# saza-ku/kube-scheduler-simulator

Measured on AMD Instinct MI355X. Metric: pods scheduled/sec @5k nodes, default plugins; node-evals/sec; % HBM peak, higher is better.
Workload: dtype int64

## Files before the change

### kube-scheduler-simulator_amd/csrc/ksched.hip

```cpp
#include <hip/hip_runtime.h>

#include <algorithm>
#include <atomic>
#include <chrono>
#include <array>
#include <cstdio>
#include <cstring>
#include <mutex>
#include <set>
#include <string>
#include <tuple>
#include <type_traits>
#include <vector>

#include "ksched_kernels.h"

#include "ksched_dev.h"
#include "ksched_json_host.h"

using namespace ksk;

#include "ksched_parts.h"

struct ksg_ctx {
// ... 671 lines not shown
    if ((rc = decide_n32(ctx, first, count, &n32))) return rc;
  }
  b.stat = n32 ? ctx->d_stat : nullptr;
  ctx->last_spec = false;
  ctx->last_mw = false;
  (void)hipGetLastError();
  treset(ctx);
  HIPC(ctx, hipEventRecord(ctx->ev0, ctx->stream));
  int trc;
  if ((trc = tmark(ctx))) return trc;
  for (int off = 0; off < count;) {
    int nb = std::min(ctx->slot_block, count - off);
    int64_t lo = 0, hi = 0;
    size_t bytes = 0;
    const size_t budget = kLdsBudget;
    for (;;) {
      lo = ctx->h_pods[first + off].blob;
      hi = lo;
      for (int k = 0; k < nb; k++) {
        const ksg_pod& q = ctx->h_pods[first + off + k];
        lo = std::min<int64_t>(lo, q.blob);
        hi = std::max<int64_t>(hi, (int64_t)q.blob + q.blob_len);
      }
      const size_t words = (cm_words + (size_t)nb * (sizeof(ksg_pod) / 4) + (size_t)(hi - lo) + 3) & ~(size_t)3;
      bytes = 4 * words + (size_t)nb * slot_bytes;
      if (bytes <= budget || nb == 1) break;
      nb = std::max(1, nb / 2);
    }
    if (bytes > budget) return fail(ctx, KSG_E_UNSUPPORTED, "batch does not fit the LDS budget");
    b.b0 = first + off;
    b.out0 = off;
    b.nb = nb;
    b.prog_lo = (int32_t)lo;
    b.prog_len = (int32_t)(hi - lo);
    const double units = (double)b.nb * N;
    hipLaunchKernelGGL(ksg_batch_phase1, dim3((N + 255) / 256, b.nb), dim3(256), 0, ctx->stream, b);
    if ((trc = tlaunched(ctx, KSG_K_BATCH_PHASE1, units))) return trc;
    hipLaunchKernelGGL(ksg_batch_topk<1024>, dim3(b.nb), dim3(1024), 0, ctx->stream, b);
    if ((trc = tlaunched(ctx, KSG_K_BATCH_TOPK, units))) return trc;
    hipLaunchKernelGGL(reinterpret_cast<void (*)(BatchArgs)>(
                           const_cast<void*>(slot_kernels()[slot_kernel_index(n32, slot_rm, ctx->slot_block)])),
                       dim3(1), dim3(ctx->slot_block), bytes, ctx->stream, b);
    if ((trc = tlaunched(ctx, KSG_K_BATCH_PHASE2S, 0.5 * b.nb * (b.nb + 1)))) return trc;
    if (cap) {
      CapArgs ca = *cap;
      ca.b0 = b.b0;
      ca.nb = b.nb;
      ca.out0 = b.out0;
      ca.rec = ctx->d_rec;
      HIPC(ctx, hipMemsetAsync(ca.stats, 0, sizeof(int32_t) * 4 * b.nb, ctx->stream));
      hipLaunchKernelGGL(ksg_capture_eval, dim3((N + 255) / 256, b.nb), dim3(256), 0, ctx->stream, ca);
      if ((trc = tlaunched(ctx, KSG_K_CAPTURE_EVAL, units))) return trc;
      hipLaunchKernelGGL(ksg_capture_norm, dim3((N + 255) / 256, b.nb), dim3(256), 0, ctx->stream, ca);
      if ((trc = tlaunched(ctx, KSG_K_CAPTURE_NORM, units))) return trc;
    }
    off += nb;
  }
  HIPC(ctx, hipGetLastError());
  HIPC(ctx, hipEventRecord(ctx->ev1, ctx->stream));
  return KSG_OK;
}

int state_copy(ksg_ctx* ctx, bool save);

int run_spec_persistent(ksg_ctx* ctx, const BatchArgs& b0, int32_t first, int32_t count, size_t cm_words, bool mw,
                        unsigned* tk, int32_t* carry_n) {
  const int N = ctx->c.N;
  constexpr int B = 64;
  std::vector<int32_t>& tab = ctx->h_btab;
  tab.clear();
  for (int off = 0, prev_nb = 0; off < count;) {
    int nb = std::min(B, count - off);
    int64_t lo = 0, hi = 0;
    size_t bytes = 0;
    for (;;) {
      lo = ctx->h_pods[first + off].blob;
      hi = lo;
      for (int k = 0; k < nb; k++) {
        const ksg_pod& q = ctx->h_pods[first + off + k];
        lo = std::min<int64_t>(lo, q.blob);
        hi = std::max<int64_t>(hi, (int64_t)q.blob + q.blob_len);
      }
      bytes = 4 * ((cm_words + (size_t)nb * (sizeof(ksg_pod) / 4) + (size_t)(hi - lo) + 3) & ~(size_t)3) +
              (size_t)kSvSlots * kSvRow * 8 + (size_t)kSvSlots * 64 * 4 + (size_t)64 * (nb + prev_nb) * 4;
      if (bytes <= kSpecLds || nb == 1) break;
      nb = std::max(1, nb / 2);
    }
    if (bytes > kSpecLds) return fail(ctx, KSG_E_UNSUPPORTED, "batch does not fit the LDS budget");
    for (int32_t v : {first + off, off, nb, (int32_t)lo, (int32_t)(hi - lo), prev_nb}) tab.push_back(v);
    prev_nb = nb;
    off += nb;
  }
  const int nbatch = (int)(tab.size() / 6);
  int rc;
  if (tab.size() > ctx->btab_cap) {
    if (ctx->d_btab) {
      auto it = std::find(ctx->allocs.begin(), ctx->allocs.end(), (void*)ctx->d_btab);
      if (it != ctx->allocs.end()) ctx->allocs.erase(it);
      HIPC(ctx, hipStreamSynchronize(ctx->stream));
      (void)hipFree(ctx->d_btab);
      ctx->d_btab = nullptr;
    }
    if ((rc = dalloc(ctx, &ctx->d_btab, tab.size()))) return rc;
    ctx->btab_cap = tab.size();
  }
  if (!ctx->h_p2done) {
    HIPC(ctx, hipHostMalloc((void**)&ctx->h_p2done, 64, hipHostMallocMapped | hipHostMallocCoherent));
    void* dp = nullptr;
    HIPC(ctx, hipHostGetDevicePointer(&dp, ctx->h_p2done, 0));
    ctx->d_p2done = static_cast<unsigned*>(dp);
  }
  hipStream_t s1 = ctx->stream2, s2 = ctx->stream;
  if ((rc = state_copy(ctx, true))) return rc;
  ctx->last_persist = true;
  HIPC(ctx, hipMemcpyAsync(ctx->d_btab, tab.data(), sizeof(int32_t) * tab.size(), hipMemcpyHostToDevice, s2));
  if (ctx->inject_timeout & 16) {
    ctx->inject_timeout &= ~16;
    HIPC(ctx, hipMemsetAsync(tk + 2, 0x01, 1, s2));
  }
  volatile unsigned* done = ctx->h_p2done;
  *done = 0;
  std::atomic_thread_fence(std::memory_order_seq_cst);
  SpecRun r{};
  r.btab = ctx->d_btab;
  r.nbatch = nbatch;
  for (int q = 0; q < 2; q++) {
    r.rec[q] = ctx->d_prec[q];
    r.img[q] = ctx->d_pimg[q];
    r.rect[q] = ctx->d_prect[q];
    r.imgt[q] = ctx->d_pimgt[q];
    r.pmax[q] = ctx->d_ppmax[q];
    r.p1[q] = ctx->d_pp1[q];
    r.top[q] = ctx->d_ptop[q];
  }
  r.carry = ctx->d_carry;
  r.carry_n = carry_n;
  r.done = ctx->d_p2done;
  BatchArgs base = b0;
  base.tk_arrive = tk;
  base.tk_done = tk + 1;
  base.tk_timeout = tk + 2;
  base.walk_err = tk + 3;
  base.inject_walk_err = ctx->inject_walk_err;
  base.tk_sc = 1;
  base.stat = nullptr;
  base.xcd_grid = 1;
  const void* run_kern = mw ? (const void*)ksg_batch_phase2v_run<64 * kSvWaves, true>
                            : (const void*)ksg_batch_phase2v_run<64 * kSvWaves, false>;
  if ((rc = func_lds_attr(ctx, run_kern, kSpecLds))) return rc;
  void* kargs[] = {&base, &r};
  HIPC(ctx, hipLaunchKernel(run_kern, dim3(1), dim3(64 * kSvWaves), kargs, kSpecLds, s2));
  const auto t0 = std::chrono::steady_clock::now();
  for (int bi = 0; bi < nbatch; bi++) {
    if (bi >= 2) {
      for (unsigned spins = 0; *done < (unsigned)(bi - 1); spins++) {
        __builtin_ia32_pause();
        if ((spins & 4095) == 4095) {
          const hipError_t e = hipStreamQuery(s2);
          if (e != hipErrorNotReady && *done < (unsigned)(bi - 1)) {
            if (e != hipSuccess) return fail(ctx, KSG_E_DEVICE, std::string("spec walk: ") + hipGetErrorString(e));
            bi = nbatch;
            break;
          }
          if (std::chrono::duration<double>(std::chrono::steady_clock::now() - t0).count() > 120.0)
            return fail(ctx, KSG_E_DEVICE, "spec walk: no progress for 120 s");
        }
      }
// ... 46 lines not shown
    }
    if ((rc = dalloc(ctx, &ctx->d_carry, (size_t)2 * KSG_BATCH_MAX + 6))) return rc;
  }
  if (!ctx->stream2) {
    int least = 0, greatest = 0;
    HIPC(ctx, hipDeviceGetStreamPriorityRange(&least, &greatest));
    HIPC(ctx, hipStreamCreateWithPriority(&ctx->stream2, hipStreamNonBlocking, greatest));
    for (int q = 0; q < 2; q++) {
      HIPC(ctx, hipEventCreateWithFlags(&ctx->ev_tk[q], hipEventDisableTiming));
      HIPC(ctx, hipEventCreateWithFlags(&ctx->ev_p2[q], hipEventDisableTiming));
    }
  }
  int32_t* carry_n = ctx->d_carry + 2 * KSG_BATCH_MAX;
  unsigned* tk = reinterpret_cast<unsigned*>(carry_n + 2);
  ctx->pipe_tk = tk;
  HIPC(ctx, hipMemsetAsync(carry_n, 0, 6 * sizeof(int32_t), ctx->stream));
  const bool window = ctx->pipe_window != 0;
  const bool overlap = window && !ctx->timing && ctx->pipe_overlap;
  const int slot_rm = ctx->c.R <= 4 ? 4 : KSG_MAX_RES;
  bool n32 = false, mw = false;
  if (ctx->batch_mode >= 4 && (rc = decide_n32(ctx, first, count, &n32))) return rc;
  if (ctx->batch_mode == 6 && window && !n32 && spec_candidate(ctx) && (rc = decide_mw(ctx, first, count, &mw)))
    return rc;
  const bool specw = ctx->batch_mode == 6 && window && (n32 || mw) && spec_candidate(ctx);
  ctx->last_spec = specw;
  ctx->last_mw = specw && mw;
  const void* spec_kern = mw ? (const void*)ksg_batch_phase2v<64 * kSvWaves, true>
                             : (const void*)ksg_batch_phase2v<64 * kSvWaves, false>;
  if (specw && !ctx->d_prect[0]) {
    for (int q = 0; q < 2; q++) {
      if ((rc = dalloc(ctx, &ctx->d_prect[q], (size_t)64 * N))) return rc;
      if ((rc = dalloc(ctx, &ctx->d_pimgt[q], (size_t)64 * N))) return rc;
    }
  }
  if (specw && (rc = func_lds_attr(ctx, spec_kern, kSpecLds))) return rc;
  const int B = specw || window ? 64 : ctx->slot_block;
  const int slots = window ? 2 * B : B;
  const int sblock = slots <= 64 ? 64 : 128;
  const void* kern = slot_kernels()[slot_kernel_index(n32, slot_rm, sblock)];
  const int block = sblock;
  const size_t kLdsBudget = specw ? kSpecLds : 120 * 1024;
  const size_t slot_bytes = 8 * (size_t)(2 * slot_rm + 10);
  if ((rc = set_phase2_attrs(ctx, 120 * 1024))) return rc;
  BatchArgs b{};
  b.c = ctx->c;
  b.st = ctx->st;
  b.pods = ctx->d_pods;
  b.prog = ctx->d_prog;
  b.prof = d_prof;
  b.placements = d_pl;
  b.results = d_res;
  const size_t cm_words = (size_t)((((N + 31) / 32) + 3) & ~3);
#ifdef KSG_STAMPS
  if (!ctx->d_stamps) {
    if ((rc = dalloc(ctx, &ctx->d_stamps, 16))) return rc;
    HIPC(ctx, hipMemsetAsync(ctx->d_stamps, 0, 128, ctx->stream));
  }
  b.stamps = ctx->d_stamps;
#endif
  hipStream_t s1 = overlap ? ctx->stream2 : ctx->stream, s2 = ctx->stream;
  (void)hipGetLastError();
  treset(ctx);
  HIPC(ctx, hipEventRecord(ctx->ev0, s2));
  if (overlap) HIPC(ctx, hipStreamWaitEvent(s1, ctx->ev0, 0));
  if ((rc = tmark(ctx))) return rc;
  if (specw && overlap && ctx->spec_persist)
    return run_spec_persistent(ctx, b, first, count, cm_words, mw, tk, carry_n);
  int prev_nb = 0;
  for (int off = 0, bi = 0; off < count; bi++) {
    const int par = bi & 1;
    int nb = std::min(B, count - off);
    int64_t lo = 0, hi = 0;
    size_t bytes = 0;
    for (;;) {
      lo = ctx->h_pods[first + off].blob;
      hi = lo;
      for (int k = 0; k < nb; k++) {
        const ksg_pod& q = ctx->h_pods[first + off + k];
        lo = std::min<int64_t>(lo, q.blob);
        hi = std::max<int64_t>(hi, (int64_t)q.blob + q.blob_len);
      }
      if (specw)
        bytes = 4 * ((cm_words + (size_t)nb * (sizeof(ksg_pod) / 4) + (size_t)(hi - lo) + 3) & ~(size_t)3) +
                (size_t)kSvSlots * kSvRow * 8 + (size_t)kSvSlots * 64 * 4 + (size_t)64 * (nb + prev_nb) * 4;
      else
        bytes = 4 * ((cm_words + (size_t)nb * (sizeof(ksg_pod) / 4) + (size_t)(hi - lo) + 3) & ~(size_t)3) +
                (size_t)sblock * slot_bytes;
      if (bytes <= kLdsBudget || nb == 1) break;
      nb = std::max(1, nb / 2);
    }
    if (bytes > kLdsBudget) return fail(ctx, KSG_E_UNSUPPORTED, "batch does not fit the LDS budget");
    b.b0 = first + off;
    b.out0 = off;
    b.nb = nb;
    b.prog_lo = (int32_t)lo;
    b.prog_len = (int32_t)(hi - lo);
    b.rec = ctx->d_prec[par];
    b.img = ctx->d_pimg[par];
    b.stat = n32 && !specw ? ctx->d_pstat[par] : nullptr;
    b.rect = specw ? ctx->d_prect[par] : nullptr;
    b.imgt = specw ? ctx->d_pimgt[par] : nullptr;
    b.xcd_grid = specw ? 1 : 0;
    b.pmax = ctx->d_ppmax[par];
    b.p1 = ctx->d_pp1[par];
    b.top = ctx->d_ptop[par];
    b.k_extra = window ? prev_nb : 0;
    b.carry = window ? ctx->d_carry + (par ^ 1) * KSG_BATCH_MAX : nullptr;
    b.carry_n = window ? carry_n + (par ^ 1) : nullptr;
    b.carry_out = window ? ctx->d_carry + par * KSG_BATCH_MAX : nullptr;
    b.carry_out_n = window ? carry_n + par : nullptr;
    const double units = (double)nb * N;
    const bool tk_flag = overlap;
    b.tk_arrive = tk_flag ? tk : nullptr;
    b.tk_done = tk_flag ? tk + 1 : nullptr;
    b.tk_timeout = tk_flag ? tk + 2 : nullptr;
    b.walk_err = tk + 3;
    b.inject_walk_err = ctx->inject_walk_err;
    b.tk_seq = (unsigned)bi + 1;
    BatchArgs bt = b;
    bt.tk_sc = specw && tk_flag ? 1 : 0;
    b.tk_sc = bt.tk_sc;
    if (overlap && bi >= 2) HIPC(ctx, hipStreamWaitEvent(s1, ctx->ev_p2[par], 0));
    if (specw)
      hipLaunchKernelGGL(ksg_batch_phase1, dim3(((((N + 255) / 256) + 7) & ~7) * nb), dim3(256), 0, s1, b);
    else
      hipLaunchKernelGGL(ksg_batch_phase1, dim3((N + 255) / 256, nb), dim3(256), 0, s1, b);
    if ((rc = tlaunched(ctx, KSG_K_BATCH_PHASE1, units))) return rc;
    hipLaunchKernelGGL(ksg_batch_topk<1024>, dim3(nb), dim3(1024), 0, s1, bt);
    if ((rc = tlaunched(ctx, KSG_K_BATCH_TOPK, units))) return rc;
    if (specw) {
      hipLaunchKernelGGL(reinterpret_cast<void (*)(BatchArgs)>(const_cast<void*>(spec_kern)), dim3(1),
                         dim3(64 * kSvWaves), kSpecLds, s2, b);
      if ((rc = tlaunched(ctx, KSG_K_BATCH_PHASE2V, 0.5 * nb * (nb + 1)))) return rc;
    } else {
      hipLaunchKernelGGL(reinterpret_cast<void (*)(BatchArgs)>(const_cast<void*>(kern)), dim3(1), dim3(block), bytes, s2, b);
      if ((rc = tlaunched(ctx, KSG_K_BATCH_PHASE2S, 0.5 * nb * (nb + 1)))) return rc;
    }
    if (overlap) HIPC(ctx, hipEventRecord(ctx->ev_p2[par], s2));
    prev_nb = nb;
    off += nb;
  }
  HIPC(ctx, hipGetLastError());
  HIPC(ctx, hipEventRecord(ctx->ev1, s2));
  return KSG_OK;
}

bool sweep_eligible(ksg_ctx* ctx, const ksg_profile* profiles, int R, int first, int count) {
  if (ctx->c.T > 255) return false;
  if (range_has_ports(ctx, first, count)) return false;
  for (int r = 0; r < R; r++) {
    const ksg_profile& prof = profiles[r];
    if (needs_topo(ctx, prof, first, count)) return false;
    int64_t wsum = 0;
    for (int pl : {KSG_PL_NODE_RESOURCES_FIT, KSG_PL_BALANCED_ALLOCATION, KSG_PL_IMAGE_LOCALITY})
      if ((prof.score_mask >> pl) & 1u) {
        if (prof.weight[pl] < 0) return false;
        wsum += prof.weight[pl];
      }
    if (wsum * 100 >= (1ll << 31)) return false;
  }
  for (int i = first; i < first + count; i++)
    if (ctx->h_na_pref_sum[i] > 0xffff || ctx->h_na_pref_sum[i] < 0) return false;
  return true;
}

template <int BLOCK, bool MULTI>
hipError_t launch_one(const void* f, const SweepArgs& s, int grid, hipStream_t st) {
// ... 2819 lines not shown
```

### kube-scheduler-simulator_amd/csrc/ksched_phase2v.h

```cpp

constexpr int kSvWaves = 12;
constexpr int kSvSlots = 2 * 64;
constexpr int kSvRow = SlotLayout<4>::STRIDE;
constexpr int kSvTotalBits = 27;
constexpr int kSvOwner = 2048;

__device__ __forceinline__ bool sv_changed(const uint32_t* cm, int n) { return ((cm[n >> 5] >> (n & 31)) & 1u) != 0; }

__device__ __forceinline__ uint32_t sv_word(int32_t total, bool live, bool p1f, bool ft, bool fa) {
  return ((uint32_t)total & ((1u << kSvTotalBits) - 1)) | (live ? 1u << 27 : 0u) | (p1f ? 1u << 28 : 0u) |
         (ft ? 1u << 29 : 0u) | (fa ? 1u << 30 : 0u) | (1u << 31);
}

struct SvItem {
  int32_t node, slot, v;
  int32_t src;
  int32_t t;
};

template <int BLOCK, bool MW = false>
__device__ __forceinline__ void spec_walk_batch(const BatchArgs& a) {
  using SL = SlotLayout<4>;
  constexpr int NW = BLOCK / 64;
  constexpr int SW = SL::W;
  static_assert(BLOCK == 64 * kSvWaves && SW == 16, "spec walk layout");
  extern __shared__ __attribute__((aligned(16))) int32_t s_dyn[];
  __shared__ ksg_profile s_prof;
  __shared__ __attribute__((aligned(16))) TcU s_u[64];
  __shared__ ksg_result s_res[64];
  __shared__ int32_t s_clist[kSvSlots];
  __shared__ int32_t s_lastv[kSvSlots];
  __shared__ int32_t s_vt[kSvSlots];
  __shared__ int32_t s_dec[64];
  __shared__ uint64_t s_bu[64];
  __shared__ uint64_t s_best[64];
  __shared__ uint32_t s_cnt[64];
  __shared__ uint8_t s_snap[64 * 64];
  __shared__ uint8_t s_mstep[64];
  __shared__ uint8_t s_dptr[64];
  __shared__ uint32_t s_owner[kSvOwner];
  __shared__ SvItem s_item[64 + 1];
  __shared__ int32_t s_ctl[8];
  __shared__ P1Stats s_p1[64];

  const int tid = threadIdx.x, lane = tid & 63, wv = tid >> 6;
  const DevCluster& c = a.c;
  const int N = c.N, R = c.R;
  const int nb = a.nb;
  const int cm_words = (((N + 31) / 32) + 3) & ~3;
  constexpr int POD_WORDS = sizeof(ksg_pod) / 4;
  const int KT = nb + a.k_extra;
  uint32_t* s_cmask = reinterpret_cast<uint32_t*>(s_dyn);
  ksg_pod* s_pods = reinterpret_cast<ksg_pod*>(s_dyn + cm_words);
  int32_t* s_prog = s_dyn + cm_words + nb * POD_WORDS;
  int64_t* s_vrow = reinterpret_cast<int64_t*>(s_dyn + ((cm_words + nb * POD_WORDS + a.prog_len + 3) & ~3));
  uint32_t* s_col = reinterpret_cast<uint32_t*>(s_vrow + (size_t)kSvSlots * kSvRow);
  int32_t* s_top = reinterpret_cast<int32_t*>(s_col + (size_t)kSvSlots * 64);

#ifdef KSG_STAMPS
  unsigned long long st_acc[16] = {}, st_last = __builtin_amdgcn_s_memtime();
#endif
  if (a.tk_done) {
    if (tid == 0) {
      using G1 = __attribute__((address_space(1))) unsigned;
      unsigned spins = 0;
      while (__hip_atomic_load((G1*)a.tk_done, __ATOMIC_RELAXED, __HIP_MEMORY_SCOPE_AGENT) < a.tk_seq) {
        __builtin_amdgcn_s_sleep(2);
        if (++spins > (1u << 24)) {
          __hip_atomic_store((G1*)a.tk_timeout, 1u, __ATOMIC_RELAXED, __HIP_MEMORY_SCOPE_AGENT);
          break;
        }
      }
    }
    __syncthreads();
    __builtin_amdgcn_fence(__ATOMIC_ACQUIRE, "agent");
  }
  KSG_STAMP(8);
  for (int i = tid; i < cm_words; i += BLOCK) s_cmask[i] = 0;
  for (int i = tid; i < kSvOwner; i += BLOCK) s_owner[i] = 0xffffffffu;
  {
    constexpr int PI = (64 * POD_WORDS + BLOCK - 1) / BLOCK;
    int32_t pw[PI];
#pragma unroll
    for (int it = 0; it < PI; it++) {
      const int i = tid + it * BLOCK;
      pw[it] = i < nb * POD_WORDS ? reinterpret_cast<const int32_t*>(a.pods + a.b0)[i] : 0;
    }
#pragma unroll
    for (int it = 0; it < PI; it++) {
      const int i = tid + it * BLOCK;
      if (i < nb * POD_WORDS) reinterpret_cast<int32_t*>(s_pods)[i] = pw[it];
    }
  }
  for (int i0 = 0; i0 < a.prog_len; i0 += 4 * BLOCK) {
    int32_t g[4];
#pragma unroll
    for (int it = 0; it < 4; it++) {
      const int i = i0 + tid + it * BLOCK;
      g[it] = i < a.prog_len ? a.prog[a.prog_lo + i] : 0;
    }
#pragma unroll
    for (int it = 0; it < 4; it++) {
      const int i = i0 + tid + it * BLOCK;
      if (i < a.prog_len) s_prog[i] = g[it];
    }
  }
  for (int i = tid; i < (int)(sizeof(ksg_profile) / 4); i += BLOCK)
    reinterpret_cast<int32_t*>(&s_prof)[i] = reinterpret_cast<const int32_t*>(a.prof)[i];
  bool fit_filter_on = false;
  for (int kf = 0; kf < a.prof->n_filter; kf++) fit_filter_on |= a.prof->filter_order[kf] == KSG_PL_NODE_RESOURCES_FIT;
  {
    const int KP = (KT + 1) >> 1;
    constexpr int TI = (64 * kSvSlots / 2 + BLOCK - 1) / BLOCK;
    ulonglong2 kp[TI];
#pragma unroll
    for (int it = 0; it < TI; it++) {
      const int x = tid + it * BLOCK, q = x / KP, i = 2 * (x - q * KP);
      const uint64_t* tp = a.top + (size_t)q * KSG_BATCH_MAX + i;
      if (x >= nb * KP) kp[it] = ulonglong2{0, 0};
      else if (a.tk_sc) kp[it] = ulonglong2{ld_sc(tp), ld_sc(tp + 1)};
      else kp[it] = *reinterpret_cast<const ulonglong2*>(tp);
    }
#pragma unroll
    for (int it = 0; it < TI; it++) {
      const int x = tid + it * BLOCK, q = x / KP, i = 2 * (x - q * KP);
      if (x < nb * KP) {
        s_top[q * KT + i] = key_node(kp[it].x);
        if (i + 1 < KT) s_top[q * KT + i + 1] = key_node(kp[it].y);
      }
    }
  }
  if (tid < nb * (int)(sizeof(P1Stats) / 4)) {
    const int32_t* src = reinterpret_cast<const int32_t*>(a.p1) + tid;
    reinterpret_cast<int32_t*>(s_p1)[tid] = a.tk_sc ? ld_sc(src) : *src;
  }
  KSG_STAMP(9);
  const int nc0 = a.carry ? *a.carry_n : 0;
  if (tid < 64) {
    const int d = a.carry && tid < nc0 ? a.carry[tid] : 0;
    if (tid < nc0) {
      s_clist[tid] = d;
      s_lastv[tid] = tid;
      s_vt[tid] = -1;
      s_item[tid] = SvItem{d, tid, tid, -1, -1};
    }
  }
  __syncthreads();
  const ksg_profile& prof = s_prof;
  const TcProf cm = tc_prof(cm_prof(prof));
  if (tid < nc0) atomicOr(&s_cmask[s_clist[tid] >> 5], 1u << (s_clist[tid] & 31));
  if (wv == 0 && lane < nb) {
    const bool ipa_filter = ipa_in_filter(prof);
    const bool ipa_score = ((prof.score_mask >> KSG_PL_INTER_POD_AFFINITY) & 1u) != 0;
    const ksg_pod& p = s_pods[lane];
    const P1Stats s1 = s_p1[lane];
    const uint32_t smask = prof.score_mask & ~p.score_skip;
    TcU u;
#pragma unroll
    for (int r = 0; r < 4; r++) u.req[r] = r < R ? p.req[r] : 0;
    u.nzc = p.nz_cpu;
    u.nzm = p.nz_mem;
    u.nfeas = s1.nfeas;
    u.K = s1.K;
    u.ht = s1.ht;
    u.ha = s1.ha;
    const bool wt = (smask & bit(KSG_PL_TAINT_TOLERATION)) && prof.weight[KSG_PL_TAINT_TOLERATION];
    const bool wa = (smask & bit(KSG_PL_NODE_AFFINITY)) && prof.weight[KSG_PL_NODE_AFFINITY];
    u.flags = (s1.err ? 1u : 0u) | (wt ? 2u : 0u) | (wa ? 4u : 0u) | (p.commit >= 0 ? 8u : 0u);
    const bool ipa_none = p.ipa < 0;
    const bool ps_skip = ipa_none && ipa_score && !((p.score_skip >> KSG_PL_INTER_POD_AFFINITY) & 1u);
    u.st_pf = ipa_none && ipa_filter ? KSG_ST_IPA_PREFILTER_SKIP : 0u;
    u.st_sc = KSG_ST_SCORED | (ps_skip ? KSG_ST_IPA_PRESCORE_SKIP : 0u);
    u.skip = p.score_skip;
    u.skip_sc = p.score_skip | (ps_skip ? bit(KSG_PL_INTER_POD_AFFINITY) : 0u);
    u.pad[0] = u.pad[1] = u.pad[2] = 0;
    s_u[lane] = u;
  }
  if (tid == 0) {
    s_ctl[0] = 0;
    s_ctl[1] = nc0;
    s_ctl[2] = nc0;
    s_ctl[3] = nc0;
    s_ctl[4] = 0;
    s_ctl[6] = 0;
  }
  __syncthreads();
  for (int q = wv; q < nb; q += NW) {
    const int K = s_u[q].K;
    int ptr = K;
    for (int b = 0; b < K && ptr == K; b += 64) {
      const int i = b + lane;
      const int n = i < K ? s_top[q * KT + i] : -1;
      const uint64_t m = __ballot(i < K && !sv_changed(s_cmask, n));
      if (m) ptr = b + __builtin_ctzll(m);
    }
    if (lane == 0) s_dptr[q] = (uint8_t)ptr;
  }
  __syncthreads();

  auto delta_word = [&](const TcU& u, int w) -> int64_t {
    const int rl = (w >> 1) & 3;
    const int64_t req_l = rl == 0 ? u.req[0] : rl == 1 ? u.req[1] : rl == 2 ? u.req[2] : u.req[3];
    return w < 8 ? ((w & 1) ? req_l : 0) : w == SL::NZC ? u.nzc : w == SL::NZM ? u.nzm : w == SL::PODS ? 1 : 0;
  };
  const int qq = lane < nb ? lane : 0;
  const TcPod hp = tc_pod(s_pods[qq], prof, s_p1[qq], fit_filter_on, R);
  struct Pending {
    SvItem it;
    uint64_t x;
    int32_t st;
    int64_t wd;
  };
  auto issue = [&](const SvItem& it) -> Pending {
    Pending p{it, 0, 0, 0};
    if (it.node < 0) return p;
    if (a.inject_walk_err && lane == 0 && it.node >= 0) {
      using G1 = __attribute__((address_space(1))) unsigned;
      __hip_atomic_store((G1*)a.walk_err, 3u, __ATOMIC_RELAXED, __HIP_MEMORY_SCOPE_AGENT);
    }
    if (it.node >= N) {
      p.it.node = -1;
      if (lane == 0) {
        using G1 = __attribute__((address_space(1))) unsigned;
        __hip_atomic_store((G1*)a.walk_err, 3u, __ATOMIC_RELAXED, __HIP_MEMORY_SCOPE_AGENT);
      }
      return p;
    }
    p.x = a.rect[(size_t)it.node * 64 + lane];
    p.st = a.imgt[(size_t)it.node * 64 + lane];
    const int wl = lane < SW ? lane : 0;
    p.wd = it.src >= 0 ? s_vrow[(size_t)it.src * kSvRow + wl]
                       : slot_word_value<4, true>(slot_word_fetch<4, true>(c, a.st, wl, R, it.node), wl, R);
    return p;
  };
  auto finish = [&](const Pending& p) {
    const SvItem& it = p.it;
    if (it.node < 0) return;
    if (lane < SW) s_vrow[(size_t)it.v * kSvRow + lane] = p.wd + (it.t >= 0 ? delta_word(s_u[it.t], lane) : 0);
    int64_t w[SW];
    {
      const int4* src = reinterpret_cast<const int4*>(s_vrow + (size_t)it.v * kSvRow);
#pragma unroll
      for (int k = 0; k < SW / 2; k++) reinterpret_cast<int4*>(w)[k] = src[k];
    }
    const TcRow row = tc_row<MW>(cm, w);
    const bool p1f = (p.x >> 63) != 0;
    const bool ft = p1f && (int32_t)((p.x >> 48) & 0xff) == hp.mt;
    const bool fa = p1f && (int32_t)((p.x >> 32) & 0xffff) == hp.ma;
    const int32_t rt = (int32_t)((p.x >> 48) & 0xff), ra = (int32_t)((p.x >> 32) & 0xffff);
    const int32_t nt = hp.mt != 0 ? 100 - qdiv32(100 * rt, hp.mt, hp.inv_mt) : 100;
    const int32_t na = hp.ma != 0 ? qdiv32(100 * ra, hp.ma, hp.inv_ma) : ra;
    const int32_t stat = p.st + hp.wt * nt + hp.wa * na;
    int32_t fb = 0;
    const bool live = tc_eval<MW>(cm, hp, row, fb) && p1f;
    if (lane > it.t) s_col[it.slot * 64 + lane] = sv_word(stat + fb, live, p1f, ft, fa);
    else if (it.src < 0) s_col[it.slot * 64 + lane] = 0u;
  };

  int ptr = 0, cnode = -1, nnode = -1;
  if (wv == 0 && lane < nb) {
    ptr = s_dptr[lane];
    const int K = s_u[lane].K;
    cnode = ptr < K ? s_top[lane * KT + ptr] : -1;
    nnode = ptr + 1 < K ? s_top[lane * KT + ptr + 1] : -1;
  }
  int start = 0, nv_c = nc0, ns_c = nc0, nspecial = nc0;
  int guard = 0;
  KSG_STAMP(0);
  while (start < nb && guard++ <= nb) {
#ifdef KSG_STAMPS
    if (tid == 0) st_acc[15] += 1;
#endif
    if (wv == 0) {
      __builtin_amdgcn_s_setprio(3);
      if (lane >= start && lane < nb) {
        s_best[lane] = 0;
        s_cnt[lane] = 0;
      }
      const int Kq = lane < nb ? s_u[lane].K : 0;
      int mi = 0;
      for (int cur = start; cur < nb; mi++) {
        s_snap[mi * 64 + lane] = (uint8_t)ptr;
        const bool act = lane >= cur && lane < nb && cnode >= 0;
        const int hsh = cnode & (kSvOwner - 1);
        if (act) atomicMin(&s_owner[hsh], (unsigned)lane);
        const unsigned o = act ? s_owner[hsh] : (unsigned)lane;
        const uint64_t dup = __ballot(act && o != (unsigned)lane);
        const int f = dup ? __builtin_ctzll(dup) : nb;
#ifdef KSG_STAMPS
        if (tid == 0) { st_acc[14] += f - cur; st_acc[12] += 1; }
#endif
        if (lane >= cur && lane < f) {
          s_dptr[lane] = (uint8_t)ptr;
          s_mstep[lane] = (uint8_t)mi;
          if (cnode >= 0) atomicOr(&s_cmask[cnode >> 5], 1u << (cnode & 31));
        }
        if (act) s_owner[hsh] = 0xffffffffu;
        if (lane == 0) {
          __atomic_signal_fence(__ATOMIC_SEQ_CST);
          __hip_atomic_store(&s_ctl[4], f - start, __ATOMIC_RELAXED, __HIP_MEMORY_SCOPE_WORKGROUP);
        }
        bool conflict = lane >= f && lane < nb && cnode >= 0 && o < (unsigned)f && sv_changed(s_cmask, cnode);
        while (__ballot(conflict)) {
#ifdef KSG_STAMPS
          if (tid == 0) st_acc[13] += 1;
#endif
          if (conflict) {
            ptr++;
            cnode = nnode;
            nnode = ptr + 1 < Kq ? s_top[lane * KT + ptr + 1] : -1;
            conflict = cnode >= 0 && sv_changed(s_cmask, cnode);
          }
        }
        cur = f;
      }
      __builtin_amdgcn_s_setprio(0);
      KSG_STAMP(1);
    }
    {
      auto take = [&](int i, bool wait, SvItem& it) -> int {
        it = SvItem{-1, 0, 0, -1, -1};
        if (i < nspecial) {
          it = s_item[i];
          return 1;
        }
        const int k = start + (i - nspecial);
        if (k >= nb) return -1;
        for (unsigned spins = 0;
             __hip_atomic_load(&s_ctl[4], __ATOMIC_RELAXED, __HIP_MEMORY_SCOPE_WORKGROUP) <= k - start; spins++) {
          if (!wait) return 0;
          if (spins >= (1u << 24)) break;
          __builtin_amdgcn_s_sleep(1);
        }
        __builtin_amdgcn_fence(__ATOMIC_ACQUIRE, "workgroup");
        const int sl = ns_c + (k - start), v = nv_c + (k - start);
        const int pk = s_dptr[k];
        const int d = pk < s_u[k].K ? s_top[k * KT + pk] : -1;
        if (lane == 0) {
          s_dec[k] = d;
          s_clist[sl] = d;
          s_lastv[sl] = v;
          s_vt[v] = k;
          const uint64_t* tp = a.top + (size_t)k * KSG_BATCH_MAX + pk;
          s_bu[k] = d < 0 ? 0 : a.tk_sc ? ld_sc(tp) : *tp;
        }
        it = SvItem{d, sl, v, -1, k};
        return 1;
      };
      auto grab = [&]() -> int {
        int i = 0;
        if (lane == 0) i = atomicAdd(&s_ctl[6], 1);
        return __builtin_amdgcn_readfirstlane(i);
      };
      SvItem ia, ib;
      int xa = grab();
      int ra = take(xa, true, ia);
      Pending pa = issue(ia), pb = issue(SvItem{-1, 0, 0, -1, -1});
      while (ra > 0) {
        const int xb = grab();
        int rb = take(xb, false, ib);
        if (rb > 0) pb = issue(ib);
        finish(pa);
        if (rb == 0) {
          rb = take(xb, true, ib);
          if (rb > 0) pb = issue(ib);
        }
        if (rb < 0) break;
        xa = grab();
        ra = take(xa, false, ia);
        if (ra > 0) pa = issue(ia);
        finish(pb);
        if (ra == 0) {
          ra = take(xa, true, ia);
          if (ra > 0) pa = issue(ia);
        }
      }
      KSG_STAMP(2);
    }
    __syncthreads();
    KSG_STAMP(3);
    {
      const int ns = ns_c + (nb - start);
      const bool mine = lane >= start && lane < nb;
      uint32_t dc = 0;
      uint64_t bk = 0;
      for (int s = wv; s < ns; s += NW) {
        const int node = s_clist[s];
        if (node < 0) continue;
        const uint32_t e = s_col[s * 64 + lane];
        const bool pres = (e >> 31) != 0;
        const bool live = pres && ((e >> 27) & 1u), p1f = pres && ((e >> 28) & 1u);
        const bool ft = (e >> 29) & 1u, fa = (e >> 30) & 1u;
        dc += (p1f ? 1u : 0u) + (live ? 1u << 8 : 0u) + (p1f && !live && ft ? 1u << 16 : 0u) +
              (p1f && !live && fa ? 1u << 24 : 0u);
        const uint64_t key = live ? argmax_key((int64_t)(e & ((1u << kSvTotalBits) - 1)), node) : 0;
        bk = key > bk ? key : bk;
      }
      if (mine && dc) atomicAdd(&s_cnt[lane], dc);
      if (mine && bk) atomicMax(reinterpret_cast<unsigned long long*>(&s_best[lane]), (unsigned long long)bk);
    }
    __syncthreads();
    KSG_STAMP(4);
    if (wv == 0) {
      const bool mine = lane < nb && lane >= start;
      const TcU u = s_u[lane < nb ? lane : 0];
      const uint32_t kc = s_cnt[lane];
      const uint64_t k0 = s_best[lane], bu = s_bu[lane];
      const int feas1 = kc & 0xff, live_n = (kc >> 8) & 0xff, lost_t = (kc >> 16) & 0xff, lost_a = kc >> 24;
      const int unch = u.nfeas - feas1;
      const int nfeas = unch + live_n;
      const bool renorm = nfeas >= 2 && ((u.flags & 1u) || ((u.flags & 2u) && u.ht - lost_t <= 0) ||
                                         ((u.flags & 4u) && u.ha - lost_a <= 0));
      int exact = -1;
      if (nfeas == 1) exact = unch == 1 ? key_node(bu) : key_node(k0);
      else if (nfeas >= 2) exact = bu > k0 ? key_node(bu) : key_node(k0);
      const int spec = s_dec[lane < nb ? lane : 0];
      const uint64_t bad = __ballot(mine && (renorm || exact != spec));
      const int ks = bad ? __builtin_ctzll(bad) : nb;
      if (mine && lane < ks) {
        const bool sc = nfeas >= 2;
        ksg_result res;
        res.selected = spec;
        res.n_feasible = nfeas;
        res.status = (sc ? KSG_ST_SCORED : 0u) | u.st_pf | (sc ? u.st_sc : 0u);
        res.score_skip = sc ? u.skip_sc : u.skip;
        s_res[lane] = res;
      }
      if (mine && lane >= ks && spec >= 0) atomicAnd(&s_cmask[spec >> 5], ~(1u << (spec & 31)));
      nv_c += ks - start;
      ns_c += ks - start;
      nspecial = 0;
      if (ks < nb) {
        const int k = ks;
        const TcU uk = s_u[k];
        const bool renorm_k = __builtin_amdgcn_readlane((int)renorm, k) != 0;
        int nfeas_k = __builtin_amdgcn_readlane(nfeas, k);
        int selected = -1;
        uint32_t status = 0;
        if (renorm_k) {
          const ksg_pod& p = s_pods[k];
          const PodView pv = make_view(c, prof, p, s_prog + (p.blob - a.prog_lo), a.prog);
          const TcPod hk = tc_pod(p, prof, s_p1[k], fit_filter_on, R);
          const uint64_t* rec = a.rec + (size_t)k * N;
          const int32_t* img = a.img + (size_t)k * N;
          auto live_rec = [&](int s) -> uint64_t {
            const int nd = s_clist[s];
            if (nd < 0) return 0;
            const uint64_t x = rec[nd];
            if (!(x >> 63)) return 0;
            int64_t w[SW];
            const int64_t* src = s_vrow + (size_t)s_lastv[s] * kSvRow;
#pragma unroll
            for (int i = 0; i < SW; i++) w[i] = src[i];
            int32_t fb = 0;
            if (!tc_eval<MW>(cm, hk, tc_row<MW>(cm, w), fb)) return 0;
            return pack_rec((int64_t)img[nd] + fb, (x >> 48) & 0xff, (x >> 32) & 0xffff);
          };
          Red r{0, 0, 0, 0x7fffffff};
          auto fold = [&](uint64_t x) {
            if (!(x >> 63)) return;
            r.nfeas += 1;
            r.max_t = max(r.max_t, (int64_t)((x >> 48) & 0xff));
            r.max_a = max(r.max_a, (int64_t)((x >> 32) & 0xffff));
          };
          for (int n = lane; n < N; n += 64)
            if (!sv_changed(s_cmask, n)) fold(rec[n]);
          for (int s = lane; s < ns_c; s += 64) fold(live_rec(s));
          const int64_t max_t = wreduce(r.max_t, OpMax64{}), max_a = wreduce(r.max_a, OpMax64{});
          nfeas_k = (int)wreduce((uint32_t)r.nfeas, OpAdd32{});
          uint64_t best = 0;
          uint32_t err = 0;
          auto visit = [&](uint64_t x, int n) {
            const int64_t rt = (x >> 48) & 0xff, ra = (x >> 32) & 0xffff, part = (uint32_t)x;
            const uint64_t key = argmax_key(total_score(pv, part, rt, ra, max_t, max_a, err, nullptr, nullptr), n);
            best = key > best ? key : best;
          };
          for (int n = lane; n < N; n += 64) {
            if (sv_changed(s_cmask, n)) continue;
            const uint64_t x = rec[n];
            if (x >> 63) visit(x, n);
          }
          for (int s = lane; s < ns_c; s += 64) {
            const uint64_t x = live_rec(s);
            if (x >> 63) visit(x, s_clist[s]);
          }
          best = wreduce(best, OpMaxU64{});
          err = wreduce(err, OpOr32{});
          status = KSG_ST_SCORED;
          if (err) status |= KSG_ST_SCORE_ERROR;
          else selected = key_node(best);
        } else {
          selected = __builtin_amdgcn_readlane(exact, k);
          status = nfeas_k >= 2 ? KSG_ST_SCORED : 0u;
        }
        int idx = -1;
        if (selected >= 0)
          for (int b = 0; b < ns_c && idx < 0; b += 64) {
            const uint64_t mk = __ballot(b + lane < ns_c && s_clist[b + lane] == selected);
            if (mk) idx = b + __builtin_ctzll(mk);
          }
        if (selected >= 0) {
          const int s = idx >= 0 ? idx : ns_c, v = nv_c;
          if (lane == 0) {
            s_item[0] = SvItem{selected, s, v, idx >= 0 ? s_lastv[idx] : -1, k};
            if (idx < 0) {
              s_clist[s] = selected;
              s_cmask[selected >> 5] |= 1u << (selected & 31);
            }
            s_lastv[s] = v;
            s_vt[v] = k;
          }
          nspecial = 1;
          nv_c += 1;
          if (idx < 0) ns_c += 1;
        }
        if (lane == 0) {
          s_dec[k] = selected;
          const bool sc = (status & KSG_ST_SCORED) != 0;
          ksg_result res;
          res.selected = selected;
          res.n_feasible = nfeas_k;
          res.status = status | uk.st_pf | (sc ? uk.st_sc : 0u);
          res.score_skip = sc ? uk.skip_sc : uk.skip;
          s_res[k] = res;
        }
        if (lane > k && lane < nb) {
          ptr = s_snap[s_mstep[k] * 64 + lane];
          cnode = ptr < u.K ? s_top[lane * KT + ptr] : -1;
          nnode = ptr + 1 < u.K ? s_top[lane * KT + ptr + 1] : -1;
          bool conflict = cnode >= 0 && sv_changed(s_cmask, cnode);
          while (conflict) {
            ptr++;
            cnode = nnode;
            nnode = ptr + 1 < u.K ? s_top[lane * KT + ptr + 1] : -1;
            conflict = cnode >= 0 && sv_changed(s_cmask, cnode);
          }
        }
      }
      if (lane == 0) {
        s_ctl[0] = ks < nb ? ks + 1 : nb;
        s_ctl[1] = nv_c;
        s_ctl[2] = ns_c;
        s_ctl[3] = nspecial;
        s_ctl[4] = 0;
        s_ctl[6] = 0;
      }
    }
    KSG_STAMP(5);
    __syncthreads();
    KSG_STAMP(6);
    start = s_ctl[0];
    nv_c = s_ctl[1];
    ns_c = s_ctl[2];
    nspecial = s_ctl[3];
  }
  if (tid == 0 && start < nb) {
    using G1 = __attribute__((address_space(1))) unsigned;
    __hip_atomic_store((G1*)a.walk_err, 2u, __ATOMIC_RELAXED, __HIP_MEMORY_SCOPE_AGENT);
  }
  if (nspecial && wv == 0) {
    const SvItem it = s_item[0];
    if (lane < SW) {
      int64_t wd = it.src >= 0 ? s_vrow[(size_t)it.src * kSvRow + lane]
                               : slot_word_value<4, true>(slot_word_fetch<4, true>(c, a.st, lane, R, it.node), lane, R);
      wd += delta_word(s_u[it.t], lane);
      s_vrow[(size_t)it.v * kSvRow + lane] = wd;
    }
  }
  __syncthreads();
  for (int x = tid; x < ns_c * SW; x += BLOCK) {
    const int s = x / SW, w = x - s * SW, node = s_clist[s];
    if (node < 0) continue;
    const int64_t val = s_vrow[(size_t)s_lastv[s] * kSvRow + w];
    if (w < 8 && (w & 1) && (w >> 1) < R) a.st.requested[(size_t)(w >> 1) * N + node] = val;
    else if (w == SL::NZC || w == SL::NZM) a.st.nonzero[(size_t)(w - SL::NZC) * N + node] = val;
    else if (w == SL::PODS) a.st.pod_count[node] = (int32_t)val;
  }
  for (int i = tid; i < nb; i += BLOCK) {
    a.placements[a.out0 + i] = s_res[i].selected;
    if (a.results) a.results[a.out0 + i] = s_res[i];
  }
  for (int i = tid; i < 2 * nb; i += BLOCK) a.pmax[i] = 0;
  uint64_t cmt = 0;
  if (wv == 0) cmt = __ballot(lane < nb && s_res[lane].selected >= 0 && (s_u[lane].flags & 8u));
  if (tid == 0 && cmt) {
    for (int k = 0; k < nb; k++) {
      if (!((cmt >> k) & 1ull)) continue;
      const int sel = s_res[k].selected;
      const ksg_pod& p = s_pods[k];
      const int32_t* cw = s_prog + (p.commit - a.prog_lo);
      const int ns = *cw++;
      for (int i = 0; i < ns; i++) a.st.cnt[(size_t)cw[i] * N + sel] += 1;
      cw += ns;
      const int nt = *cw++;
      for (int i = 0; i < nt; i++) {
        const int t = cw[2 * i];
        const uint32_t lv = c.label_val[(size_t)c.tmpl_col[t] * N + sel];
        if (!lv) continue;
        a.st.tab[c.tmpl_off[t] + lv] += c.tmpl_kind[t] == KSG_TMPL_PREF ? cw[2 * i + 1] : 1;
        a.st.tmpl_total[t] += 1;
      }
    }
  }
  if (a.carry_out && wv == 0) {
    int base = 0;
    for (int b = 0; b < ns_c; b += 64) {
      const int s = b + lane;
      const bool t = s < ns_c && s_clist[s] >= 0 && s_vt[s_lastv[s]] >= 0;
      const uint64_t m = __ballot(t);
      if (t) a.carry_out[base + __popcll(m & ((1ull << lane) - 1))] = s_clist[s];
      base += __popcll(m);
    }
    if (lane == 0) *a.carry_out_n = base;
  }
  KSG_STAMP(7);
#ifdef KSG_STAMPS
  if (tid == 0 && a.stamps)
    for (int i = 0; i < 16; i++) atomicAdd(&a.stamps[i], st_acc[i]);
#endif
}

template <int BLOCK, bool MW = false>
__global__ __launch_bounds__(BLOCK) void ksg_batch_phase2v(BatchArgs a) {
  spec_walk_batch<BLOCK, MW>(a);
}

struct SpecRun {
  const int32_t* btab;
  int32_t nbatch;
  uint64_t* rec[2];
  int32_t* img[2];
  uint64_t* rect[2];
  int32_t* imgt[2];
  int32_t* pmax[2];
  P1Stats* p1[2];
  uint64_t* top[2];
  int32_t* carry;
  int32_t* carry_n;
  unsigned* done;
};

template <int BLOCK, bool MW = false>
__global__ __launch_bounds__(BLOCK) void ksg_batch_phase2v_run(BatchArgs base, SpecRun r) {
  __shared__ int s_stop;
  using G1 = __attribute__((address_space(1))) unsigned;
  for (int bi = 0; bi < r.nbatch; bi++) {
    BatchArgs a = base;
    const int32_t* d = r.btab + 6 * bi;
    a.b0 = d[0];
    a.out0 = d[1];
    a.nb = d[2];
    a.prog_lo = d[3];
// ... 29 lines not shown
```

### profiles/stamps.py

```python
import ctypes as C
import importlib
import os
import sys

ROOT = os.path.dirname(os.path.dirname(os.path.abspath(__file__)))
sys.path.insert(0, ROOT)
G = importlib.import_module("kube-scheduler-simulator_amd.generator")
E = importlib.import_module("kube-scheduler-simulator_amd.encoder")
native = importlib.import_module("kube-scheduler-simulator_amd.native")

n_pods = int(sys.argv[1]) if len(sys.argv) > 1 else 10000
if len(sys.argv) > 2 and sys.argv[2] == "default":
    nodes, pods, prof = G.config1(n_nodes=5000, n_pods=n_pods)
else:
    nodes, pods, prof = G.config2(n_pods=n_pods)
enc = E.Encoder(nodes, pods, prof)
eng = native.Engine(lib_path=os.path.join(ROOT, "kube-scheduler-simulator_amd", "libksched_stamps.so"))
eng.load(enc, E.encode_profile(prof, enc.cluster.res_names))
eng.run_queue(0, n_pods, results=False)
ms = eng.last_kernel_ms()
st = (C.c_ulonglong * 16)()
fn = eng.lib.ksg_debug_stamps
fn.argtypes = [C.c_void_p, C.c_void_p]
assert fn(eng.ctx, st) == 0
tot = sum(st[1:])
mode = os.environ.get("KSG_BATCH_MODE", "pipe")
if mode == "pipe":
    names = ["(unused)", "bu + candidate buffer reads", "evaluate pod j+1 (both versions)",
             "candidates of pod j+1 + loads", "fold + decide", "contributions (reductions)",
             "results (lane 0)", "assume + record rotation", "candidate stores (wait for loads)", "barrier"]
    print(f"[pipe] {n_pods} pods, kernel {ms:.1f} ms, {ms * 1e3 / n_pods:.2f} us/pod (stamped build)")
    tot = sum(st[1:10])
    for i in range(1, 10):
        print(f"  {names[i]:36s} {st[i] / n_pods:10.0f} cycles/pod  {100 * st[i] / tot:5.1f} %")
    sys.exit(0)
if mode == "tcol":
    names = ["(loop top)", "rescan check + P1 reads", "decide", "assume + result", "next-pod candidate + loads",
             "row read", "column eval + running maxima"]
    print(f"[tcol] {n_pods} pods, kernel {ms:.1f} ms, {ms * 1e3 / n_pods:.2f} us/pod (stamped build)")
    tot = sum(st[0:7])
    for i in range(0, 7):
        print(f"  {names[i]:36s} {st[i] / n_pods:10.0f} cycles/pod  {100 * st[i] / tot:5.1f} %")
    sys.exit(0)
if mode == "spec":
    names = ["setup (LDS staging, initial pointers)", "S: speculate + publish (wave 0)", "V: wave 0 verifying after S",
             "barrier (other waves still verifying)", "A: aggregate + barrier", "C: check + commit (wave 0)",
             "barrier", "epilogue"]
    print(f"[spec] {n_pods} pods, kernel {ms:.1f} ms, {ms * 1e3 / n_pods:.2f} us/pod (stamped build); "
          f"rounds per batch {st[15] / max(1, (n_pods + 63) // 64):.2f}, speculation steps per batch "
          f"{st[14] / max(1, (n_pods + 63) // 64):.1f} in {st[12] / max(1, (n_pods + 63) // 64):.1f} macro-steps, "
          f"step-on iterations per batch {st[13] / max(1, (n_pods + 63) // 64):.1f}")
    names += ["setup: wait for phase 1 / top-k", "setup: staging (pods, programs, T)"]
    names[0] = "setup: carried slots, pod records, initial pointers"
    tot = sum(st[0:10])
    for i in (8, 9, 0, 1, 2, 3, 4, 5, 6, 7):
        print(f"  {names[i]:40s} {st[i] / n_pods:10.0f} cycles/pod  {100 * st[i] / tot:5.1f} %")
    sys.exit(0)
if mode in ("slot", "window"):
    names = ["(start)", "X: speculate + issue next-pod loads", "X: changed node + DPP reductions",
             "Y: barrier 1 + decide (+renorm)", "Y: row update + results", "barrier 2",
             "Y: next-pod records + top set (waits)", "Y: fetched column decode"]
else:
    names = ["(start)", "A: changed nodes + top sets", "barrier 1", "B: decide (+rescan)",
             "B: next-pod LDS writes", "barrier 2 (waits for the assume)"]
print(f"[{mode}] {n_pods} pods, kernel {ms:.1f} ms, {ms * 1e3 / n_pods:.2f} us/pod (stamped build)")
if mode in ("slot", "window") and any(st[8:13]):
    names += [""] * 8
    names[8], names[9], names[1] = "X0: pod setup (LDS pod/P1 reads)", "X1: speculated node (top set, C)", "X2: issue next-pod loads"
    names[10], names[11], names[12] = "X3a: to slot evaluation", "X3b: slot read + Fit/BA scores", "X3c: normalise + key"
    names[2] = "X3d: DPP reductions + partials"
    for i in (8, 9, 1, 10, 11, 12, 2, 3, 6, 7, 4, 5):
        print(f"  {names[i]:36s} {st[i] / n_pods:10.0f} cycles/pod  {100 * st[i] / tot:5.1f} %")
    sys.exit(0)
for i in range(1, 8 if mode in ("slot", "window") else 6):
    print(f"  {names[i]:36s} {st[i] / n_pods:10.0f} cycles/pod  {100 * st[i] / tot:5.1f} %")
```

Baseline: 988,100.

## Keep unaffected speculated pods across rollbacks in spec walk

```diff
diff --git a/kube-scheduler-simulator_amd/csrc/ksched.hip b/kube-scheduler-simulator_amd/csrc/ksched.hip
--- a/kube-scheduler-simulator_amd/csrc/ksched.hip
+++ b/kube-scheduler-simulator_amd/csrc/ksched.hip
@@ -777,7 +777,7 @@
         hi = std::max<int64_t>(hi, (int64_t)q.blob + q.blob_len);
       }
       bytes = 4 * ((cm_words + (size_t)nb * (sizeof(ksg_pod) / 4) + (size_t)(hi - lo) + 3) & ~(size_t)3) +
-              (size_t)kSvSlots * kSvRow * 8 + (size_t)kSvSlots * 64 * 4 + (size_t)64 * (nb + prev_nb) * 4;
+              (size_t)kSvSlots * kSvRow * 8 + (size_t)kSvSlots * 64 * 4 + (size_t)64 * ((nb + prev_nb) | 1) * 4;
       if (bytes <= kSpecLds || nb == 1) break;
       nb = std::max(1, nb / 2);
     }
@@ -990,7 +990,7 @@
       }
       if (specw)
         bytes = 4 * ((cm_words + (size_t)nb * (sizeof(ksg_pod) / 4) + (size_t)(hi - lo) + 3) & ~(size_t)3) +
-                (size_t)kSvSlots * kSvRow * 8 + (size_t)kSvSlots * 64 * 4 + (size_t)64 * (nb + prev_nb) * 4;
+                (size_t)kSvSlots * kSvRow * 8 + (size_t)kSvSlots * 64 * 4 + (size_t)64 * ((nb + prev_nb) | 1) * 4;
       else
         bytes = 4 * ((cm_words + (size_t)nb * (sizeof(ksg_pod) / 4) + (size_t)(hi - lo) + 3) & ~(size_t)3) +
                 (size_t)sblock * slot_bytes;
diff --git a/kube-scheduler-simulator_amd/csrc/ksched_phase2v.h b/kube-scheduler-simulator_amd/csrc/ksched_phase2v.h
--- a/kube-scheduler-simulator_amd/csrc/ksched_phase2v.h
+++ b/kube-scheduler-simulator_amd/csrc/ksched_phase2v.h
@@ -40,6 +40,7 @@
   __shared__ uint8_t s_dptr[64];
   __shared__ uint32_t s_owner[kSvOwner];
   __shared__ SvItem s_item[64 + 1];
+  __shared__ int32_t s_evnode[64];
   __shared__ int32_t s_ctl[8];
   __shared__ P1Stats s_p1[64];
 
@@ -49,7 +50,8 @@
   const int nb = a.nb;
   const int cm_words = (((N + 31) / 32) + 3) & ~3;
   constexpr int POD_WORDS = sizeof(ksg_pod) / 4;
-  const int KT = nb + a.k_extra;
+  const int KN = nb + a.k_extra;
+  const int KT = KN | 1;
   uint32_t* s_cmask = reinterpret_cast<uint32_t*>(s_dyn);
   ksg_pod* s_pods = reinterpret_cast<ksg_pod*>(s_dyn + cm_words);
   int32_t* s_prog = s_dyn + cm_words + nb * POD_WORDS;
@@ -110,7 +112,7 @@
   bool fit_filter_on = false;
   for (int kf = 0; kf < a.prof->n_filter; kf++) fit_filter_on |= a.prof->filter_order[kf] == KSG_PL_NODE_RESOURCES_FIT;
   {
-    const int KP = (KT + 1) >> 1;
+    const int KP = (KN + 1) >> 1;
     constexpr int TI = (64 * kSvSlots / 2 + BLOCK - 1) / BLOCK;
     ulonglong2 kp[TI];
 #pragma unroll
@@ -126,7 +128,7 @@
       const int x = tid + it * BLOCK, q = x / KP, i = 2 * (x - q * KP);
       if (x < nb * KP) {
         s_top[q * KT + i] = key_node(kp[it].x);
-        if (i + 1 < KT) s_top[q * KT + i + 1] = key_node(kp[it].y);
+        if (i + 1 < KN) s_top[q * KT + i + 1] = key_node(kp[it].y);
       }
     }
   }
@@ -138,6 +140,7 @@
   const int nc0 = a.carry ? *a.carry_n : 0;
   if (tid < 64) {
     const int d = a.carry && tid < nc0 ? a.carry[tid] : 0;
+    s_evnode[tid] = -1;
     if (tid < nc0) {
       s_clist[tid] = d;
       s_lastv[tid] = tid;
@@ -178,8 +181,8 @@
   }
   if (tid == 0) {
     s_ctl[0] = 0;
-    s_ctl[1] = nc0;
-    s_ctl[2] = nc0;
+    s_ctl[1] = 0;
+    s_ctl[2] = 0;
     s_ctl[3] = nc0;
     s_ctl[4] = 0;
     s_ctl[6] = 0;
@@ -253,6 +256,9 @@
     const int32_t stat = p.st + hp.wt * nt + hp.wa * na;
     int32_t fb = 0;
     const bool live = tc_eval<MW>(cm, hp, row, fb) && p1f;
+#ifdef KSG_STAMPS
+    if (lane == 0 && a.stamps) atomicAdd(&a.stamps[10], 1ull);
+#endif
     if (lane > it.t) s_col[it.slot * 64 + lane] = sv_word(stat + fb, live, p1f, ft, fa);
     else if (it.src < 0) s_col[it.slot * 64 + lane] = 0u;
   };
@@ -264,7 +270,7 @@
     cnode = ptr < K ? s_top[lane * KT + ptr] : -1;
     nnode = ptr + 1 < K ? s_top[lane * KT + ptr + 1] : -1;
   }
-  int start = 0, nv_c = nc0, ns_c = nc0, nspecial = nc0;
+  int start = 0, rs = 0, mi0 = 0, nspecial = nc0;
   int guard = 0;
   KSG_STAMP(0);
   while (start < nb && guard++ <= nb) {
@@ -278,8 +284,8 @@
         s_cnt[lane] = 0;
       }
       const int Kq = lane < nb ? s_u[lane].K : 0;
-      int mi = 0;
-      for (int cur = start; cur < nb; mi++) {
+      int mi = mi0;
+      for (int cur = rs; cur < nb; mi++) {
         s_snap[mi * 64 + lane] = (uint8_t)ptr;
         const bool act = lane >= cur && lane < nb && cnode >= 0;
         const int hsh = cnode & (kSvOwner - 1);
@@ -324,7 +330,7 @@
           it = s_item[i];
           return 1;
         }
-        const int k = start + (i - nspecial);
+        const int k = rs + (i - nspecial);
         if (k >= nb) return -1;
         for (unsigned spins = 0;
              __hip_atomic_load(&s_ctl[4], __ATOMIC_RELAXED, __HIP_MEMORY_SCOPE_WORKGROUP) <= k - start; spins++) {
@@ -333,10 +339,12 @@
           __builtin_amdgcn_s_sleep(1);
         }
         __builtin_amdgcn_fence(__ATOMIC_ACQUIRE, "workgroup");
-        const int sl = ns_c + (k - start), v = nv_c + (k - start);
+        const int sl = nc0 + k, v = nc0 + k;
         const int pk = s_dptr[k];
         const int d = pk < s_u[k].K ? s_top[k * KT + pk] : -1;
+        if (d >= 0 && s_evnode[k] == d) return 1;
         if (lane == 0) {
+          s_evnode[k] = d;
           s_dec[k] = d;
           s_clist[sl] = d;
           s_lastv[sl] = v;
@@ -380,7 +388,7 @@
     __syncthreads();
     KSG_STAMP(3);
     {
-      const int ns = ns_c + (nb - start);
+      const int ns = nc0 + nb;
       const bool mine = lane >= start && lane < nb;
       uint32_t dc = 0;
       uint64_t bk = 0;
@@ -427,11 +435,11 @@
         s_res[lane] = res;
       }
       if (mine && lane >= ks && spec >= 0) atomicAnd(&s_cmask[spec >> 5], ~(1u << (spec & 31)));
-      nv_c += ks - start;
-      ns_c += ks - start;
       nspecial = 0;
+      int q1 = nb, m0 = 0;
       if (ks < nb) {
         const int k = ks;
+        const int ns_c = nc0 + k;
         const TcU uk = s_u[k];
         const bool renorm_k = __builtin_amdgcn_readlane((int)renorm, k) != 0;
         int nfeas_k = __builtin_amdgcn_readlane(nfeas, k);
@@ -499,8 +507,12 @@
             const uint64_t mk = __ballot(b + lane < ns_c && s_clist[b + lane] == selected);
             if (mk) idx = b + __builtin_ctzll(mk);
           }
+        if (lane == 0) {
+          s_clist[ns_c] = -1;
+          s_evnode[k] = -1;
+        }
         if (selected >= 0) {
-          const int s = idx >= 0 ? idx : ns_c, v = nv_c;
+          const int s = idx >= 0 ? idx : ns_c, v = ns_c;
           if (lane == 0) {
             s_item[0] = SvItem{selected, s, v, idx >= 0 ? s_lastv[idx] : -1, k};
             if (idx < 0) {
@@ -511,8 +523,6 @@
             s_vt[v] = k;
           }
           nspecial = 1;
-          nv_c += 1;
-          if (idx < 0) ns_c += 1;
         }
         if (lane == 0) {
           s_dec[k] = selected;
@@ -524,12 +534,40 @@
           res.score_skip = sc ? uk.skip_sc : uk.skip;
           s_res[k] = res;
         }
-        if (lane > k && lane < nb) {
-          ptr = s_snap[s_mstep[k] * 64 + lane];
+        const int Y = __builtin_amdgcn_readlane(spec, k);
+        const bool later = lane > k && lane < nb;
+        int posY = -1;
+        if (later && Y >= 0 && Y != selected) {
+          const int dp = min((int)s_dptr[lane], kSvSlots);
+#pragma unroll 4
+          for (int i = s_snap[s_mstep[k] * 64 + lane]; i < dp; i++) posY = s_top[lane * KT + i] == Y ? i : posY;
+        }
+        const uint64_t am = __ballot(later && (posY >= 0 || (selected >= 0 && idx < 0 && spec == selected)));
+        q1 = am ? __builtin_ctzll(am) : nb;
+        int row = s_mstep[q1 < nb ? q1 : k];
+        m0 = row + 1;
+        const bool full = q1 < nb && m0 + (nb - q1) > 64;
+        if (full) {
+          q1 = k + 1;
+          m0 = 0;
+          row = s_mstep[k];
+        }
+#ifdef KSG_STAMPS
+        if (tid == 0) st_acc[11] += q1 - (k + 1);
+#endif
+        if (lane > k && lane < q1 && spec >= 0) atomicOr(&s_cmask[spec >> 5], 1u << (spec & 31));
+        if (lane >= q1 && lane < nb) {
+          ptr = s_snap[row * 64 + lane];
+          if (posY >= 0) {
+            ptr = min(ptr, posY);
+            if (!full)
+              for (int m = s_mstep[k]; m <= row && m < 64; m++)
+                if (s_snap[m * 64 + lane] > posY) s_snap[m * 64 + lane] = (uint8_t)posY;
+          }
           cnode = ptr < u.K ? s_top[lane * KT + ptr] : -1;
           nnode = ptr + 1 < u.K ? s_top[lane * KT + ptr + 1] : -1;
           bool conflict = cnode >= 0 && sv_changed(s_cmask, cnode);
-          while (conflict) {
+          for (int g = 0; conflict && g < kSvSlots; g++) {
             ptr++;
             cnode = nnode;
             nnode = ptr + 1 < u.K ? s_top[lane * KT + ptr + 1] : -1;
@@ -539,10 +577,10 @@
       }
       if (lane == 0) {
         s_ctl[0] = ks < nb ? ks + 1 : nb;
-        s_ctl[1] = nv_c;
-        s_ctl[2] = ns_c;
+        s_ctl[1] = q1;
+        s_ctl[2] = m0;
         s_ctl[3] = nspecial;
-        s_ctl[4] = 0;
+        s_ctl[4] = ks < nb ? q1 - (ks + 1) : 0;
         s_ctl[6] = 0;
       }
     }
@@ -550,8 +588,8 @@
     __syncthreads();
     KSG_STAMP(6);
     start = s_ctl[0];
-    nv_c = s_ctl[1];
-    ns_c = s_ctl[2];
+    rs = s_ctl[1];
+    mi0 = s_ctl[2];
     nspecial = s_ctl[3];
   }
   if (tid == 0 && start < nb) {
@@ -568,6 +606,7 @@
     }
   }
   __syncthreads();
+  const int ns_c = nc0 + nb;
   for (int x = tid; x < ns_c * SW; x += BLOCK) {
     const int s = x / SW, w = x - s * SW, node = s_clist[s];
     if (node < 0) continue;
diff --git a/profiles/stamps.py b/profiles/stamps.py
--- a/profiles/stamps.py
+++ b/profiles/stamps.py
@@ -49,7 +49,9 @@
     print(f"[spec] {n_pods} pods, kernel {ms:.1f} ms, {ms * 1e3 / n_pods:.2f} us/pod (stamped build); "
           f"rounds per batch {st[15] / max(1, (n_pods + 63) // 64):.2f}, speculation steps per batch "
           f"{st[14] / max(1, (n_pods + 63) // 64):.1f} in {st[12] / max(1, (n_pods + 63) // 64):.1f} macro-steps, "
-          f"step-on iterations per batch {st[13] / max(1, (n_pods + 63) // 64):.1f}")
+          f"step-on iterations per batch {st[13] / max(1, (n_pods + 63) // 64):.1f}, row versions evaluated per batch "
+          f"{st[10] / max(1, (n_pods + 63) // 64):.1f}, pods kept across rollbacks per batch "
+          f"{st[11] / max(1, (n_pods + 63) // 64):.1f}")
     names += ["setup: wait for phase 1 / top-k", "setup: staging (pods, programs, T)"]
     names[0] = "setup: carried slots, pod records, initial pointers"
     tot = sum(st[0:10])
```

New measurement: 1.065 million (median of 6 runs). 1.08x the previous value.
